# Audio-WestlakeU/SAR-SSL

Hardware: AMD Instinct MI355X
Metric: pretrain_segments_per_sec (higher is better)
Workload: dtype fp16 stem + f32 residual stream (fp16-pair MFMA operands: hi hi + lo hi + hi lo), bf16 backward

## Files before the change

sar-ssl_amd/csrc/conv3x3.hip:

```cpp
#include "common.h"
#include <stdlib.h>

#define TR 8
#define TCOL 64
#define HR (TR + 2)
#define HC (TCOL + 2)
#define NPIX_H (HR * HC)
#define NCHUNK_H (NPIX_H * 8)
#define X_ITERS 11
#define W_ELEMS (9 * 64 * 64)
#define X_ELEMS (NPIX_H * 64)
#define Y_ELEMS (TR * TCOL * 64)

struct ConvArgs {
    const void* in; const void* w; void* out;
    float* acc_ws; int acc_in, acc_out;
    const float* scale; const float* shift; int prologue;
    int nb, F, T;
    int part_in, part_w;
    double* stats;
    const void* bn_y;
    const float* bn_aff;
    int prio;
    const float* c1_w;
// ... 655 lines not shown
    volatile __attribute__((address_space(3))) unsigned* ready3 = (volatile __attribute__((address_space(3))) unsigned*)&sReady[half];
    for (int it = 0; it < nrounds; ++it) {
        const int tile = tile_of(it);
        if (tile >= ntiles) break;
        const TileCoord tc = coord(tile);
        while (*ready3 < (unsigned)(it + 1) * 4u) __builtin_amdgcn_s_sleep(1);
        asm volatile("" ::: "memory");

        f32x16 acc[2][2];
#pragma unroll
        for (int i = 0; i < 2; ++i)
#pragma unroll
            for (int j = 0; j < 2; ++j)
#pragma unroll
                for (int r = 0; r < 16; ++r) acc[i][j][r] = 0.f;
        {
            bf16x8 wf[2][2], xf[2][2];
            auto fetch = [&](int s, int buf) {
                const int tap = s >> 2, kc = s & 3;
                const int kh = tap / 3, kw = tap - kh * 3;
#pragma unroll
                for (int i = 0; i < 2; ++i) wf[buf][i] = *(const bf16x8*)(sW + laneW[kc] + (tap * 64 + i * 32) * 64);
#pragma unroll
                for (int j = 0; j < 2; ++j) xf[buf][j] = *(const bf16x8*)(sX + laneX[kw][kc] + ((kh + j) * PHC) * 64);
            };
            if (a.prio) __builtin_amdgcn_s_setprio(3);
            fetch(0, 0);
#pragma unroll
            for (int s = 0; s < 36; ++s) {
                const int cur = s & 1;
                if (s + 1 < 36) fetch(s + 1, cur ^ 1);
                __builtin_amdgcn_sched_barrier(0);
#pragma unroll
                for (int i = 0; i < 2; ++i)
#pragma unroll
                    for (int j = 0; j < 2; ++j)
                        acc[i][j] = mfma16<bf16>(wf[cur][i], xf[cur][j], acc[i][j]);
            }
            if (a.prio) __builtin_amdgcn_s_setprio(0);
        }
        __builtin_amdgcn_s_waitcnt(0x0F70);
        uint2 av[2];
        bool pv[2];
#pragma unroll
        for (int j = 0; j < 2; ++j) {
            const int f = tc.f0 + 2 * hw + j, t = tc.t0 + (lane & 31);
            pv[j] = f < F && t < Tn;
            av[j] = *(const uint2*)((const uint16_t*)a.c1_a0 + (((long)tc.b * F + min(f, F - 1)) * Tn + min(t, Tn - 1)) * 4);
        }
        half_barrier(cnt, epoch, lane);
        uint16_t* stg = sX + hw * (64 * 64);
        __builtin_amdgcn_s_waitcnt(0x0F70);
        if constexpr (!__is_same(TY, bf16)) {
#pragma unroll
            for (int j = 0; j < 2; ++j) {
                av[j].x = pack2_bf16(H16<TY>::lo(av[j].x), H16<TY>::hi(av[j].x));
                av[j].y = pack2_bf16(H16<TY>::lo(av[j].y), H16<TY>::hi(av[j].y));
            }
        }
        uint16_t* a0t = sX + 4 * (64 * 64) + hw * 256;
        {
            const int j = lane >> 5;
            const uint2 q = j ? av[1] : av[0];
            uint16_t* d = a0t + j * 32 + (lane & 31);
            d[0] = (uint16_t)(q.x & 0xffffu); d[64] = (uint16_t)(q.x >> 16); d[128] = (uint16_t)(q.y & 0xffffu); d[192] = (uint16_t)(q.y >> 16);
        }
#pragma unroll
        for (int i = 0; i < 2; ++i) {
            const bf16x8 wfr = *(const bf16x8*)&sC1[(i * 32 + (lane & 31)) * 16 + (lane >> 5) * 8];
#pragma unroll
            for (int j = 0; j < 2; ++j) {
                union { uint4 u; bf16x8 b; } bx;
                bx.u = make_uint4(av[j].x, av[j].y, 0x00003f80u, 0u);
                f32x16 y;
#pragma unroll
                for (int r = 0; r < 16; ++r) y[r] = 0.f;
                y = __builtin_amdgcn_mfma_f32_32x32x16_bf16(wfr, bx.b, y, 0, 0, 0);
#pragma unroll
                for (int r = 0; r < 16; ++r) acc[i][j][r] = (y[r] > 0.f && pv[j]) ? acc[i][j][r] : 0.f;
            }
        }
#pragma unroll
        for (int i = 0; i < 2; ++i)
#pragma unroll
            for (int g = 0; g < 4; ++g)
#pragma unroll
                for (int j = 0; j < 2; ++j) {
                    uint2 w2;
                    w2.x = pack2_bf16(acc[i][j][g * 4 + 0], acc[i][j][g * 4 + 1]);
                    w2.y = pack2_bf16(acc[i][j][g * 4 + 2], acc[i][j][g * 4 + 3]);
                    *(uint2*)(stg + swz(j * 32 + (lane & 31), i * 4 + g) + 4 * (lane >> 5)) = w2;
                }
        __builtin_amdgcn_s_waitcnt(0xC07F);
        __builtin_amdgcn_wave_barrier();
        f32x16 d2[2];
#pragma unroll
        for (int nb = 0; nb < 2; ++nb)
#pragma unroll
            for (int r = 0; r < 16; ++r) d2[nb][r] = 0.f;
        const int m = lane & 31;
#pragma unroll
        for (int ks = 0; ks < 4; ++ks) {
            union { uint4 u; bf16x8 b; } ax;
            ax.u = *(const uint4*)(a0t + min(m, 3) * 64 + ks * 16 + (lane >> 5) * 8);
            if (m == 4) ax.u = make_uint4(0x3f803f80u, 0x3f803f80u, 0x3f803f80u, 0x3f803f80u);
            else if (m > 4) ax.u = make_uint4(0u, 0u, 0u, 0u);
#pragma unroll
            for (int nb = 0; nb < 2; ++nb)
                d2[nb] = __builtin_amdgcn_mfma_f32_32x32x16_bf16(ax.b, tr_frag(stg, ks * 16, nb * 32, lane), d2[nb], 0, 0, 0);
        }
#pragma unroll
        for (int nb = 0; nb < 2; ++nb)
#pragma unroll
            for (int r = 0; r < 4; ++r) gacc[nb][r] += d2[nb][r];
        __builtin_amdgcn_s_waitcnt(0xC07F);
        if (lane == 0) atomicAdd(&sFree[half], 1u);
    }
    __syncthreads();
    if (a.clk && blockIdx.x == 0 && tid == 0) { a.clk[2] = __builtin_amdgcn_s_memtime(); a.clk[3] = __builtin_amdgcn_s_memrealtime(); }
    float* fold = (float*)sW + 1024;
#pragma unroll
    for (int nb = 0; nb < 2; ++nb) {
        const int co = nb * 32 + (lane & 31);
        if (lane < 32) {
#pragma unroll
            for (int r = 0; r < 4; ++r) fold[wave * 320 + co * 4 + r] = gacc[nb][r];
        } else fold[wave * 320 + 256 + co] = gacc[nb][0];
    }
    __syncthreads();
    for (int q = tid; q < 320; q += 512) {
        float s = 0.f;
#pragma unroll
        for (int w = 0; w < 8; ++w) s += fold[w * 320 + q];
        atomicAdd(&a.c1_red[q < 256 ? q : 512 + (q - 256)], (double)s);
    }
}

struct WgradArgs {
    const void* dy;
    const void* zin;
    const float* scale; const float* shift; int prologue;
    float* partial;
    int nb, F, T;
    int part_dy, part_z;
    const float* c1_w;
    const void* y;
    const float* aff;
    const double* red;
    int use_stats;
    void* dy_out;
    const void* dy4;
    const float* W4;
    float* pg_w4; float* pg_gamma; float* pg_beta;
};
enum { DY_LOAD = 0, DY_APPLY = 1, DY_C4 = 2 };

__device__ __forceinline__ int swzc(int p, int col, int chunk) { return (p * 8 + (chunk ^ (((col >> 1) & 1) << 2))) * 8; }
__device__ __forceinline__ bf16x8 tr_pair(const uint16_t* p0, const uint16_t* p1) {
    typedef __attribute__((ext_vector_type(4))) short s16x4;
    union { s16x4 v[2]; bf16x8 b; } u;
    u.v[0] = __builtin_amdgcn_ds_read_tr16_b64_v4i16((__attribute__((address_space(3))) s16x4*)p0);
    u.v[1] = __builtin_amdgcn_ds_read_tr16_b64_v4i16((__attribute__((address_space(3))) s16x4*)p1);
    return u.b;
}

__global__ __launch_bounds__(512) void conv3x3_wgrad_kernel(WgradArgs a) {
    __shared__ __attribute__((aligned(16))) uint16_t sY[Y_ELEMS];
    __shared__ __attribute__((aligned(16))) uint16_t sX[X_ELEMS];
    const int tid = threadIdx.x, lane = tid & 63, wave = tid >> 6;
    const int wi = wave & 1, wj = (wave >> 1) & 1, wt = wave >> 2;
    const int tap0 = wt ? 5 : 0, ntap = wt ? 4 : 5;
    const int F = a.F, Tn = a.T;
    const int tiles_f = (F + TR - 1) / TR, tiles_t = (Tn + TCOL - 1) / TCOL;
    const int ntiles = a.nb * tiles_f * tiles_t;
    const float* zin = (const float*)a.zin;
    const float* dy = (const float*)a.dy;
    const int cch = tid & 7;

    f32x16 acc[5];
#pragma unroll
    for (int t9 = 0; t9 < 5; ++t9)
#pragma unroll
        for (int r = 0; r < 16; ++r) acc[t9][r] = 0.f;

    int baseA[2], baseB[5][2];
    {
        const int chA = wi * 32 + 16 * ((lane >> 4) & 1) + (lane & 3) * 4, chB = wj * 32 + 16 * ((lane >> 4) & 1) + (lane & 3) * 4;
#pragma unroll
        for (int h = 0; h < 2; ++h) {
            const int loff = (lane >> 5) * 8 + h * 4 + ((lane & 15) >> 2);
            baseA[h] = swzc(loff, loff, chA >> 3) + (chA & 7);
#pragma unroll
            for (int tt = 0; tt < 5; ++tt) {
                const int tap = tap0 + (tt < ntap ? tt : 0);
                const int kh = tap / 3, kw = tap - kh * 3;
                baseB[tt][h] = swzc(kh * HC + kw + loff, kw + loff, chB >> 3) + (chB & 7);
            }
        }
    }

    Chunk<float> rz[X_ITERS], ry[8];
    const int pc = tid >> 3;
    auto issue_loads = [&](int tile) {
        const TileCoord tc = tile_coord(tile, tiles_f, tiles_t);
        const int t = tc.t0 - 1 + pc;
#pragma unroll
        for (int i = 0; i < HR; ++i) rz[i] = load_chunk_clamped<float>(zin, tc.b, tc.f0 - 1 + i, t, F, Tn, cch * 8);
        {
            const int hr = pc >> 1, te = tc.t0 + TCOL - 1 + (pc & 1);
            rz[HR] = load_chunk_clamped<float>(zin, tc.b, tc.f0 - 1 + hr, te, F, Tn, cch * 8);
        }
        const int ty = tc.t0 + pc;
#pragma unroll
        for (int i = 0; i < 8; ++i) ry[i] = load_chunk_clamped<float>(dy, tc.b, tc.f0 + i, ty, F, Tn, cch * 8);
    };
    auto write_tile = [&](int tile) {
        const TileCoord tc = tile_coord(tile, tiles_f, tiles_t);
        float sc[8], sh[8];
#pragma unroll
        for (int e = 0; e < 8; ++e) { sc[e] = a.prologue ? a.scale[cch * 8 + e] : 1.f; sh[e] = a.prologue ? a.shift[cch * 8 + e] : 0.f; }
        const int t = tc.t0 - 1 + pc;
        const bool tv = t >= 0 && t < Tn;
#pragma unroll
        for (int i = 0; i < HR; ++i) {
            const int f = tc.f0 - 1 + i;
            *(uint4*)&sX[swzc(i * HC + pc, pc, cch)] = xform_chunk<float>(rz[i], tv && f >= 0 && f < F, a.prologue, sc, sh, a.part_z);
        }
        if (tid < 160) {
            const int hr = pc >> 1, f = tc.f0 - 1 + hr, te = tc.t0 + TCOL - 1 + (pc & 1);
            *(uint4*)&sX[swzc(hr * HC + TCOL + (pc & 1), TCOL + (pc & 1), cch)] = xform_chunk<float>(rz[HR], f >= 0 && f < F && te < Tn, a.prologue, sc, sh, a.part_z);
        }
        const int ty = tc.t0 + pc;
#pragma unroll
        for (int i = 0; i < 8; ++i)
            *(uint4*)&sY[swzc(i * 64 + pc, pc, cch)] = xform_chunk<float>(ry[i], tc.f0 + i < F && ty < Tn, 0, sc, sh, a.part_dy);
    };

    const int nrounds = (ntiles + gridDim.x - 1) / gridDim.x;
    if (xcd_tile(0, blockIdx.x, gridDim.x) < ntiles) issue_loads(xcd_tile(0, blockIdx.x, gridDim.x));
    for (int it = 0; it < nrounds; ++it) {
        const int tile = xcd_tile(it, blockIdx.x, gridDim.x);
        if (tile >= ntiles) break;
        write_tile(tile);
        __syncthreads();
        const int next = (it + 1 < nrounds) ? xcd_tile(it + 1, blockIdx.x, gridDim.x) : ntiles;
        if (next < ntiles) issue_loads(next);
#pragma unroll 1
        for (int r = 0; r < TR; ++r) {
            const uint16_t* ya[2] = {sY + baseA[0] + r * (64 * 64), sY + baseA[1] + r * (64 * 64)};
            const uint16_t* xb[5][2];
#pragma unroll
            for (int tt = 0; tt < 5; ++tt) { xb[tt][0] = sX + baseB[tt][0] + r * (HC * 64); xb[tt][1] = sX + baseB[tt][1] + r * (HC * 64); }
#pragma unroll
            for (int cb = 0; cb < 4; ++cb) {
                const int co_ = cb * 16 * 64;
                const bf16x8 fa = tr_pair(ya[0] + co_, ya[1] + co_);
                bf16x8 fb[2];
                fb[0] = tr_pair(xb[0][0] + co_, xb[0][1] + co_);
#pragma unroll
                for (int tt = 0; tt < 5; ++tt) {
                    if (tt + 1 < 5 && tt + 1 < ntap) fb[(tt + 1) & 1] = tr_pair(xb[tt + 1][0] + co_, xb[tt + 1][1] + co_);
                    __builtin_amdgcn_sched_barrier(0);
                    if (tt < ntap) acc[tt] = __builtin_amdgcn_mfma_f32_32x32x16_bf16(fa, fb[tt & 1], acc[tt], 0, 0, 0);
                }
            }
        }
        __syncthreads();
    }
    float* P = a.partial + (long)blockIdx.x * W_ELEMS;
#pragma unroll
    for (int tt = 0; tt < 5; ++tt) {
        if (tt < ntap) {
            const int tap = tap0 + tt;
#pragma unroll
            for (int r = 0; r < 16; ++r) {
                const int co = wi * 32 + (r & 3) + 8 * (r >> 2) + 4 * (lane >> 5);
                const int ci = wj * 32 + (lane & 31);
                P[(tap * 64 + co) * 64 + ci] = acc[tt][r];
            }
        }
    }
}

#define WTC 32
#define WHC (WTC + 2)
#define WX_ELEMS (HR * WHC * 64)
#define WY_ELEMS (TR * WTC * 64)
template <bool C1IN = false, typename TA = bf16, int DYSRC = DY_LOAD, typename TY = bf16>
__global__ __launch_bounds__(1024) void conv3x3_wgrad_ws_kernel(WgradArgs a) {
    typedef bf16 T;
    __shared__ __attribute__((aligned(16))) uint16_t sYb[2][WY_ELEMS];
    __shared__ __attribute__((aligned(16))) uint16_t sXb[2][WX_ELEMS];
    constexpr int KROWS = DYSRC == DY_C4 ? 8 : 5, KZ = KROWS * 64;
    static_assert(sizeof(C1Const) == 40 * sizeof(float), "C1Const layout");
    __shared__ __attribute__((aligned(16))) float sK[DYSRC == DY_LOAD ? 4 : KZ + (C1IN ? 8 * 40 : 2 * 64)];
    const int lane = threadIdx.x & 63;
    const int wave_all = __builtin_amdgcn_readfirstlane(threadIdx.x >> 6);
    const bool producer = wave_all >= 8;
    const int tid = threadIdx.x & 511;
    const int wave = wave_all & 7;
    const int wi = wave & 1, wj = (wave >> 1) & 1, wt = wave >> 2;
    const int tap0 = wt ? 5 : 0, ntap = wt ? 4 : 5;
    const int F = a.F, Tn = a.T;
    const int tiles_f = (F + TR - 1) / TR, tiles_t = (Tn + WTC - 1) / WTC;
    const int ntiles = a.nb * tiles_f * tiles_t;
    const TA* zin = (const TA*)a.zin;
    const T* dy = (const T*)a.dy;
    const int cch = tid & 7;

    const int nrounds = (ntiles + gridDim.x - 1) / gridDim.x;
    int tile = xcd_tile(0, blockIdx.x, gridDim.x);
    if (producer) {
        float sc[8], sh[8];
        C1Const kc1;
        if constexpr (DYSRC == DY_LOAD) {
    #pragma unroll
            for (int e = 0; e < 8; ++e) { sc[e] = a.prologue ? a.scale[cch * 8 + e] : 1.f; sh[e] = a.prologue ? a.shift[cch * 8 + e] : 0.f; }
            if (C1IN) c1_setup(kc1, a.c1_w, a.scale, a.shift, cch * 8);
        }
        auto load_z = [&](int b, int f, int t) __attribute__((always_inline)) {
            Chunk<TA> c;
            if (C1IN) {
                f = min(max(f, 0), F - 1); t = min(max(t, 0), Tn - 1);
                const uint2 q = *(const uint2*)(zin + (((long)b * F + f) * Tn + t) * 4);
                c.u = make_uint4(q.x, q.y, 0u, 0u);
            } else c = load_chunk_clamped<TA>(zin, b, f, t, F, Tn, cch * 8);
            return c;
        };
        auto xform_z = [&](const Chunk<TA>& c, bool ok) __attribute__((always_inline)) { return C1IN ? c1_chunk<TA, bf16>(c.u.x, c.u.y, ok, kc1) : xform_chunk<TA, bf16>(c, ok, a.prologue, sc, sh, 0); };

        Chunk<TA> rz[6]; Chunk<T> ry[4];
        Chunk<TY> rv[4]; uint2 rd[4];
        const int pcol = (tid >> 3) & 31;
        const int pr = __builtin_amdgcn_readfirstlane(tid >> 8);
        const int lbX = swzc(pr * WHC + pcol, pcol, cch), lbY = swzc(pr * WTC + pcol, pcol, cch);
        auto coord = [&](int tile) __attribute__((always_inline)) { TileCoord c; c.t0 = (tile % tiles_t) * WTC; tile /= tiles_t; c.f0 = (tile % tiles_f) * TR; c.b = tile / tiles_f; return c; };
        auto issue_loads = [&](const TileCoord tc) __attribute__((always_inline)) {
            constexpr unsigned PXB = C1IN ? 8u : 128u;
            const char* zimg = (const char*)zin + (long)tc.b * F * (long)Tn * PXB;
            const char* yimg = (const char*)dy + (long)tc.b * F * (long)Tn * 128;
            const unsigned zrow = (unsigned)Tn * PXB, yrow = (unsigned)Tn * 128u;
            const int tz = min(max(tc.t0 - 1 + pcol, 0), Tn - 1), ty = min(tc.t0 + pcol, Tn - 1);
            const unsigned vz = C1IN ? (unsigned)tz * 8u : (unsigned)(tz * 64 + cch * 8) * 2u, vy = (unsigned)(ty * 64 + cch * 8) * 2u;
    #pragma unroll
            for (int k = 0; k < 5; ++k) {
                const int f = min(max(tc.f0 - 1 + pr + 2 * k, 0), F - 1);
                const char* prow = zimg + (unsigned)f * zrow;
                if (C1IN) { const uint2 q = *(const uint2*)(prow + vz); rz[k].u = make_uint4(q.x, q.y, 0u, 0u); }
                else rz[k].u = *(const uint4*)(prow + vz);
            }
            {
                const int q = tid >> 3, hr = q >> 1, te = tc.t0 + WTC - 1 + (q & 1);
                rz[5] = load_z(tc.b, tc.f0 - 1 + hr, te);
            }
            const char* vimg = (const char*)a.y + (long)tc.b * F * (long)Tn * 128;
            const char* dcol = (const char*)a.dy4 + ((long)tc.b * Tn + ty) * (long)F * 8;
    #pragma unroll
            for (int k = 0; k < 4; ++k) {
                const int f = min(tc.f0 + pr + 2 * k, F - 1);
                if constexpr (DYSRC != DY_C4) ry[k].u = *(const uint4*)(yimg + (unsigned)f * yrow + vy);
                if constexpr (DYSRC != DY_LOAD) rv[k].u = *(const uint4*)(vimg + (unsigned)f * yrow + vy);
                if constexpr (DYSRC == DY_C4) rd[k] = *(const uint2*)(dcol + (unsigned)f * 8u);
            }
        };
        auto write_piece = [&](const int piece, const TileCoord tc, uint16_t* __restrict__ sX, uint16_t* __restrict__ sY) __attribute__((always_inline)) {
            if (piece < 2) {
                const int t = tc.t0 - 1 + pcol;
                const bool tv = t >= 0 && t < Tn;
    #pragma unroll
                for (int k = 0; k < 5; ++k) {
                    if ((piece == 0) != (k < 3)) continue;
                    const int f = tc.f0 - 1 + pr + 2 * k;
                    *(uint4*)&sX[lbX + k * (2 * WHC * 64)] = xform_z(rz[k], tv && f >= 0 && f < F);
                    }
                if (piece == 1 && tid < 160) {
                    const int q = tid >> 3, hr = q >> 1, f = tc.f0 - 1 + hr, te = tc.t0 + WTC - 1 + (q & 1);
                    *(uint4*)&sX[swzc(hr * WHC + WTC + (q & 1), WTC + (q & 1), cch)] = xform_z(rz[5], f >= 0 && f < F && te < Tn);
                }
            } else {
                const int ty = tc.t0 + pcol;
                if constexpr (DYSRC == DY_LOAD) {
    #pragma unroll
                    for (int k = 0; k < 4; ++k) {
                        *(uint4*)&sY[lbY + k * (2 * WTC * 64)] = xform_chunk<T>(ry[k], tc.f0 + pr + 2 * k < F && ty < Tn, 0, sc, sh, 0);
                    }
                } else {
                    uint32_t o[4][4];
                    constexpr int NE = DYSRC == DY_C4 ? 2 : 4;
                    auto word = [](const uint4& u, int i) __attribute__((always_inline)) { return i == 0 ? u.x : i == 1 ? u.y : i == 2 ? u.z : u.w; };
    #pragma unroll
                    for (int h = 0; h < 8 / NE; ++h) {
                        const int c0 = cch * 8 + h * NE;
                        __builtin_amdgcn_sched_barrier(0);
                        auto row = [&](int r, float* v) __attribute__((always_inline)) {
                            if constexpr (NE == 4) { const float4 q = *(const float4*)&sK[r * 64 + c0]; v[0] = q.x; v[1] = q.y; v[2] = q.z; v[3] = q.w; }
                            else { const float2 q = *(const float2*)&sK[r * 64 + c0]; v[0] = q.x; v[1] = q.y; }
                        };
                        float kA[NE], kB[NE], kC[NE];
                        if constexpr (DYSRC == DY_APPLY) {
                            float thr[NE], sf[NE];
                            row(0, kA); row(1, kB); row(2, kC); row(3, thr); row(4, sf);
                            unsigned sgn = 0u;
    #pragma unroll
                            for (int e = 0; e < NE; ++e) sgn |= __float_as_uint(sf[e]) << e;
    #pragma unroll
                            for (int k = 0; k < 4; ++k) {
                                float d[NE], y[NE], r[NE];
    #pragma unroll
                                for (int j = 0; j < NE / 2; ++j) {
                                    const uint32_t dw = word(ry[k].u, h * (NE / 2) + j), yw = word(rv[k].u, h * (NE / 2) + j);
                                    d[2 * j] = H16<T>::lo(dw); d[2 * j + 1] = H16<T>::hi(dw);
                                    y[2 * j] = H16<TY>::lo(yw); y[2 * j + 1] = H16<TY>::hi(yw);
                                }
                                bn_bwd_apply_relu<NE>(d, y, kA, kB, kC, thr, sgn, r);
    #pragma unroll
                                for (int j = 0; j < NE / 2; ++j) {
                                    o[k][h * (NE / 2) + j] = pack2_bf16(r[2 * j], r[2 * j + 1]);
                                    asm volatile("" : "+v"(o[k][h * (NE / 2) + j]));
                                }
                            }
                        } else {
                            float w0[NE], w1[NE], w2[NE], w3[NE], s3[NE], h3[NE];
                            row(0, w0); row(1, w1); row(2, w2); row(3, w3); row(4, s3); row(5, h3); row(6, kB); row(7, kC);
    #pragma unroll
                            for (int k = 0; k < 4; ++k) {
                                float y[NE], r[NE];
    #pragma unroll
                                for (int j = 0; j < NE / 2; ++j) {
                                    const uint32_t yw = word(rv[k].u, h * (NE / 2) + j);
                                    y[2 * j] = H16<TY>::lo(yw); y[2 * j + 1] = H16<TY>::hi(yw);
                                }
                                const float4 d4 = make_float4(H16<T>::lo(rd[k].x), H16<T>::hi(rd[k].x), H16<T>::lo(rd[k].y), H16<T>::hi(rd[k].y));
                                stem_c4_bwd_apply<NE>(y, d4, w0, w1, w2, w3, s3, h3, s3, kB, kC, r);
    #pragma unroll
                                for (int j = 0; j < NE / 2; ++j) {
                                    o[k][h * (NE / 2) + j] = pack2_bf16(r[2 * j], r[2 * j + 1]);
                                    asm volatile("" : "+v"(o[k][h * (NE / 2) + j]));
                                }
                            }
                        }
                    }
                    char* oimg = (char*)a.dy_out + (long)tc.b * F * (long)Tn * 128;
                    const unsigned yrow = (unsigned)Tn * 128u, vy = (unsigned)(ty * 64 + cch * 8) * 2u;
    #pragma unroll
                    for (int k = 0; k < 4; ++k) {
                        const int f = tc.f0 + pr + 2 * k;
                        const bool ok = f < F && ty < Tn;
                        const uint4 u = ok ? make_uint4(o[k][0], o[k][1], o[k][2], o[k][3]) : make_uint4(0, 0, 0, 0);
                        *(uint4*)&sY[lbY + k * (2 * WTC * 64)] = u;
                        if (ok) *(uint4*)(oimg + (unsigned)f * yrow + vy) = u;
                    }
                }
            }
        };
        auto write_tile = [&](const TileCoord tc, uint16_t* __restrict__ sX, uint16_t* __restrict__ sY) __attribute__((always_inline)) {
            if constexpr (DYSRC != DY_LOAD) {
                if constexpr (C1IN) kc1 = *(const C1Const*)&sK[KZ + cch * 40];
                else {
    #pragma unroll
                    for (int e = 0; e < 8; ++e) { sc[e] = sK[KZ + cch * 8 + e]; sh[e] = sK[KZ + 64 + cch * 8 + e]; }
                }
            }
            write_piece(0, tc, sX, sY); write_piece(1, tc, sX, sY); write_piece(2, tc, sX, sY);
        };

        TileCoord tc = coord(tile < ntiles ? tile : 0);
        if (tile < ntiles) issue_loads(tc);
        if constexpr (DYSRC != DY_LOAD) {
            constexpr int RO = DYSRC == DY_C4 ? 256 : 0;
            if (blockIdx.x == 0 && a.pg_gamma) {
                if (DYSRC == DY_C4 && tid < 256) a.pg_w4[tid] += (float)a.red[tid];
                if (tid < 64) { a.pg_beta[tid] += (float)a.red[RO + tid]; a.pg_gamma[tid] += (float)a.red[RO + 64 + tid]; }
            }
            if (tid < 64) {
                const float invN = 1.0f / (float)((long)a.nb * F * Tn);
                const float s_ = a.aff[tid], h_ = a.aff[64 + tid], mu = a.aff[128 + tid], rs = a.aff[192 + tid];
                const float m1 = a.use_stats ? (float)a.red[RO + tid] * invN : 0.f, m2 = a.use_stats ? (float)a.red[RO + 64 + tid] * invN : 0.f;
                float A, B, C;
                bn_bwd_abc(s_, mu, rs, m1, m2, A, B, C);
                if constexpr (DYSRC == DY_APPLY) {
                    bool neg;
                    const float t = bn_relu_thr(s_, h_, neg);
                    sK[tid] = A; sK[64 + tid] = B; sK[128 + tid] = C; sK[192 + tid] = t; sK[256 + tid] = __uint_as_float(neg ? 1u : 0u);
                } else {
    #pragma unroll
                    for (int c = 0; c < 4; ++c) sK[c * 64 + tid] = a.W4[c * 64 + tid];
                    sK[256 + tid] = s_; sK[320 + tid] = h_; sK[384 + tid] = B; sK[448 + tid] = C;
                }
                if constexpr (C1IN) {
                    if (tid < 8) { C1Const k; c1_setup(k, a.c1_w, a.scale, a.shift, tid * 8); *(C1Const*)&sK[KZ + tid * 40] = k; }
                } else { sK[KZ + tid] = a.prologue ? a.scale[tid] : 1.f; sK[KZ + 64 + tid] = a.prologue ? a.shift[tid] : 0.f; }
            }
            __syncthreads();
        }
        if (tile < ntiles) write_tile(tc, sXb[0], sYb[0]);
        int next = (1 < nrounds) ? xcd_tile(1, blockIdx.x, gridDim.x) : ntiles;
        TileCoord tcn = coord(next < ntiles ? next : 0);
        if (next < ntiles) issue_loads(tcn);
        __syncthreads();
        int cur = 0;
        for (int it = 0; it < nrounds; ++it) {
            if (tile >= ntiles) break;
            if (next < ntiles) write_tile(tcn, sXb[cur ^ 1], sYb[cur ^ 1]);
            const int nn = (it + 2 < nrounds) ? xcd_tile(it + 2, blockIdx.x, gridDim.x) : ntiles;
            const TileCoord tcnn = coord(nn < ntiles ? nn : 0);
            if (nn < ntiles) issue_loads(tcnn);
            __syncthreads();
            cur ^= 1; tile = next; next = nn; tcn = tcnn;
        }
        return;
    }
    f32x16 acc[5];
#pragma unroll
    for (int t9 = 0; t9 < 5; ++t9)
#pragma unroll
        for (int r = 0; r < 16; ++r) acc[t9][r] = 0.f;

    int baseA[2], baseB[5][2];
    {
        const int chA = wi * 32 + 16 * ((lane >> 4) & 1) + (lane & 3) * 4, chB = wj * 32 + 16 * ((lane >> 4) & 1) + (lane & 3) * 4;
#pragma unroll
        for (int h = 0; h < 2; ++h) {
            const int loff = (lane >> 5) * 8 + h * 4 + ((lane & 15) >> 2);
            baseA[h] = swzc(loff, loff, chA >> 3) + (chA & 7);
#pragma unroll
            for (int tt = 0; tt < 5; ++tt) {
                const int tap = tap0 + (tt < ntap ? tt : 0);
                const int kh = tap / 3, kw = tap - kh * 3;
                baseB[tt][h] = swzc(kh * WHC + kw + loff, kw + loff, chB >> 3) + (chB & 7);
            }
        }
    }
    if constexpr (DYSRC != DY_LOAD) __syncthreads();
    __syncthreads();
    int cur = 0;
    for (int it = 0; it < nrounds; ++it) {
        if (tile >= ntiles) break;
        const int next = (it + 1 < nrounds) ? xcd_tile(it + 1, blockIdx.x, gridDim.x) : ntiles;
        const uint16_t* sX = sXb[cur];
        const uint16_t* sY = sYb[cur];
#pragma unroll
        for (int r = 0; r < TR; ++r) {
            const uint16_t* ya[2] = {sY + baseA[0] + r * (WTC * 64), sY + baseA[1] + r * (WTC * 64)};
            const uint16_t* xb[5][2];
#pragma unroll
            for (int tt = 0; tt < 5; ++tt) { xb[tt][0] = sX + baseB[tt][0] + r * (WHC * 64); xb[tt][1] = sX + baseB[tt][1] + r * (WHC * 64); }
#pragma unroll
            for (int cb = 0; cb < WTC / 16; ++cb) {
                const int co_ = cb * 16 * 64;
                const bf16x8 fa = tr_pair(ya[0] + co_, ya[1] + co_);
                bf16x8 fb[2];
                fb[0] = tr_pair(xb[0][0] + co_, xb[0][1] + co_);
#pragma unroll
                for (int tt = 0; tt < 5; ++tt) {
                    if (tt + 1 < 5 && tt + 1 < ntap) fb[(tt + 1) & 1] = tr_pair(xb[tt + 1][0] + co_, xb[tt + 1][1] + co_);
                    __builtin_amdgcn_sched_barrier(0);
                    if (tt < ntap) acc[tt] = __builtin_amdgcn_mfma_f32_32x32x16_bf16(fa, fb[tt & 1], acc[tt], 0, 0, 0);
                }
            }
        }
        __syncthreads();
        cur ^= 1; tile = next;
    }
    float* P = a.partial + (long)blockIdx.x * W_ELEMS;
#pragma unroll
    for (int tt = 0; tt < 5; ++tt) {
        if (tt < ntap) {
            const int tap = tap0 + tt;
#pragma unroll
            for (int r = 0; r < 16; ++r) {
                const int co = wi * 32 + (r & 3) + 8 * (r >> 2) + 4 * (lane >> 5);
                const int ci = wj * 32 + (lane & 31);
                P[(tap * 64 + co) * 64 + ci] = acc[tt][r];
            }
        }
    }
}

__global__ __launch_bounds__(256) void wgrad_reduce_kernel(const float* __restrict__ partial, int nparts, float* __restrict__ dW,
                                                           int accumulate, float* __restrict__ grad_oihw = nullptr) {
    __shared__ float sred[4][64];
    const int col = threadIdx.x & 63, slot = threadIdx.x >> 6;
    const int e = blockIdx.x * 64 + col;
    float s0 = 0.f, s1 = 0.f, s2 = 0.f, s3 = 0.f;
    int p = slot;
    for (; p + 12 < nparts; p += 16) {
        s0 += partial[(long)p * W_ELEMS + e]; s1 += partial[(long)(p + 4) * W_ELEMS + e];
        s2 += partial[(long)(p + 8) * W_ELEMS + e]; s3 += partial[(long)(p + 12) * W_ELEMS + e];
    }
    for (; p < nparts; p += 4) s0 += partial[(long)p * W_ELEMS + e];
    sred[slot][col] = (s0 + s1) + (s2 + s3);
    __syncthreads();
    if (slot == 0) {
        const float t = (sred[0][col] + sred[1][col]) + (sred[2][col] + sred[3][col]);
        if (grad_oihw) { const int tap = e >> 12, coci = e & 4095; grad_oihw[coci * 9 + tap] += t; }
        else dW[e] = accumulate ? dW[e] + t : t;
    }
}

static int conv_cus_override() { const sarssl_ctx* c = sarssl_current(); return c ? c->conv_cus_bwd : 0; }
static int conv_cus(int kind) {
    const int ncu = sarssl_cu_count();
    const int ovr = conv_cus_override();
    if (kind == 1 && ovr > 0) return ovr < ncu ? ovr : ncu;
    return kind == 1 && ncu >= 64 ? (ncu * 7 / 8) & ~7 : ncu;
}
static unsigned long long* conv_clk() { const sarssl_ctx* c = sarssl_current(); return c ? c->conv_clk : nullptr; }
extern "C" long sarssl_wall_clock_khz() {
    int khz = 0;
    if (hipDeviceGetAttribute(&khz, hipDeviceAttributeWallClockRate, 0) != hipSuccess) return 0;
    return (long)khz;
}
static int conv_persistent_grid(int nunits, int kind) {
    const int cus = conv_cus(kind);
    if (nunits <= cus) return nunits;
    const int rounds = (nunits + cus - 1) / cus;
    int g = (nunits + rounds - 1) / rounds;
    g = (g + 7) & ~7;
    return g < cus ? g : cus;
}
static int wgrad_db_grid(int nb, int F, int T) {
    const int ntiles = nb * ((F + TR - 1) / TR) * ((T + WTC - 1) / WTC);
    return conv_persistent_grid(ntiles, 1);
}
static int conv_grid(int nb, int F, int T) {
    int ntiles = nb * ((F + TR - 1) / TR) * ((T + TCOL - 1) / TCOL);
    const int ncu = sarssl_cu_count();
    return ntiles < ncu ? ntiles : ncu;
}
static int conv_npairs(int nb, int F, int T) { return (nb * ((F + TR - 1) / TR) * ((T + PTC - 1) / PTC) + 1) / 2; }
static ConvArgs conv_args(const void* in, const void* w, void* out, int nb, int F, int T, int clk_slot) {
    ConvArgs a = {};
#ifdef CONV_STAMPS
    a.stamps = g_conv_stamps_host;
#endif
    a.prio = (sarssl_mfma_prio() == 1 || sarssl_mfma_prio() == 2);
    a.clk = conv_clk() ? conv_clk() + 4 * clk_slot : nullptr;
    a.in = in; a.w = w; a.out = out;
    a.nb = nb; a.F = F; a.T = T;
    return a;
}

static int conv3x3_launch(const void* in, const void* w, void* out, int dtype, int w_dtype, int nb, int F, int T,
                          const float* scale, const float* shift, int precise, float* ws, double* stats, const void* bn_y,
                          const float* bn_aff, void* stream, int y_dtype = SARSSL_BF16);

extern "C" int sarssl_conv3x3_fwd(const void* in, const void* w, void* out, int dtype, int w_dtype, int nb, int F, int T,
                                  const float* scale, const float* shift, int precise, float* ws, double* stats, void* stream) {
    return conv3x3_launch(in, w, out, dtype, w_dtype, nb, F, T, scale, shift, precise, ws, stats, nullptr, nullptr, stream);
}

extern "C" int sarssl_conv3x3_dgrad_bnred(const void* dy, const void* w, void* dz, int nb, int F, int T, const void* y,
                                          const float* aff, double* red, int y_dtype, void* stream) {
    SARSSL_REQUIRE(y != nullptr && aff != nullptr && red != nullptr && (y_dtype == SARSSL_BF16 || y_dtype == SARSSL_F16), "sarssl_conv3x3_dgrad_bnred");
    return conv3x3_launch(dy, w, dz, SARSSL_BF16, SARSSL_BF16, nb, F, T, nullptr, nullptr, 0, nullptr, red, y, aff, stream, y_dtype);
}

extern "C" int sarssl_conv3x3_fwd_c1(const void* a0, const float* W1, const float* scale, const float* shift, const void* w, void* out,
                                     int nb, int F, int T, double* stats, int dtype, void* stream) {
    SARSSL_REQUIRE(nb > 0 && F > 0 && T > 0 && a0 && W1 && scale && shift && (dtype == SARSSL_BF16 || dtype == SARSSL_F16), "sarssl_conv3x3_fwd_c1");
    if (stats && SARSSL_ZERO(stats, 128 * sizeof(double), (hipStream_t)stream) != hipSuccess) { sarssl_set_error("memset"); return -2; }
    ConvArgs a = conv_args(a0, w, out, nb, F, T, 3);
    a.stats = stats;
    a.scale = scale; a.shift = shift; a.prologue = 1; a.c1_w = W1;
    const int g = conv_persistent_grid(conv_npairs(nb, F, T), 0);
    if (dtype == SARSSL_F16) conv3x3_fwd_pp_kernel<false, true, f16><<<g, 512, 0, (hipStream_t)stream>>>(a);
    else conv3x3_fwd_pp_kernel<false, true><<<g, 512, 0, (hipStream_t)stream>>>(a);
    SARSSL_CHECK_LAUNCH("conv3x3_fwd_pp_kernel<c1in>");
    return 0;
}

extern "C" int sarssl_conv3x3_dgrad_c1red(const void* dy, const void* w, const void* a0, const float* W1, const float* scale,
                                          const float* shift, int nb, int F, int T, double* red, int a0_dtype, void* stream) {
    SARSSL_REQUIRE(nb > 0 && F > 0 && T > 0 && dy && w && a0 && W1 && scale && shift && red && (a0_dtype == SARSSL_BF16 || a0_dtype == SARSSL_F16),
                   "sarssl_conv3x3_dgrad_c1red");
    if (SARSSL_ZERO(red, 644 * sizeof(double), (hipStream_t)stream) != hipSuccess) { sarssl_set_error("memset"); return -2; }
    ConvArgs a = conv_args(dy, w, nullptr, nb, F, T, 4);
    a.scale = scale; a.shift = shift; a.c1_w = W1; a.c1_a0 = a0; a.c1_red = red;
    const int g = conv_persistent_grid(conv_npairs(nb, F, T), 1);
    if (a0_dtype == SARSSL_F16) conv3x3_dgrad_c1red_ws_kernel<f16><<<g, 768, 0, (hipStream_t)stream>>>(a);
    else conv3x3_dgrad_c1red_ws_kernel<bf16><<<g, 768, 0, (hipStream_t)stream>>>(a);
    SARSSL_CHECK_LAUNCH("conv3x3_dgrad_c1red_ws_kernel");
    return 0;
}

static int conv3x3_launch(const void* in, const void* w, void* out, int dtype, int w_dtype, int nb, int F, int T,
                          const float* scale, const float* shift, int precise, float* ws, double* stats, const void* bn_y,
                          const float* bn_aff, void* stream, int y_dtype) {
    SARSSL_REQUIRE(nb > 0 && F > 0 && T > 0, "sarssl_conv3x3_fwd");
    SARSSL_REQUIRE(stats == nullptr || dtype == SARSSL_BF16 || dtype == SARSSL_F16, "sarssl_conv3x3_fwd(fused statistics: 16-bit storage only)");
    if (stats && SARSSL_ZERO(stats, 128 * sizeof(double), (hipStream_t)stream) != hipSuccess) { sarssl_set_error("memset"); return -2; }
    ConvArgs a = conv_args(in, w, out, nb, F, T, bn_y ? 2 : (scale != nullptr ? 0 : 1));
    a.bn_y = bn_y; a.bn_aff = bn_aff;
    a.stats = stats;
    a.scale = scale; a.shift = shift; a.prologue = (scale != nullptr);
    hipStream_t st = (hipStream_t)stream;
    if (dtype == w_dtype && (dtype == SARSSL_BF16 || dtype == SARSSL_F16)) {
        const int g = conv_persistent_grid(conv_npairs(nb, F, T), scale != nullptr ? 0 : 1);
        if (dtype == SARSSL_F16) {
            SARSSL_REQUIRE(bn_y == nullptr, "sarssl_conv3x3_fwd(fp16: forward launches only)");
            conv3x3_fwd_pp_kernel<false, false, f16><<<g, 512, 0, st>>>(a);
        } else if (bn_y && y_dtype == SARSSL_F16) conv3x3_fwd_pp_kernel<true, false, bf16, f16><<<g, 512, 0, st>>>(a);
        else if (bn_y) conv3x3_fwd_pp_kernel<true><<<g, 512, 0, st>>>(a);
        else conv3x3_fwd_pp_kernel<false><<<g, 512, 0, st>>>(a);
    } else if (dtype == SARSSL_F32 && w_dtype == SARSSL_F32) {
        const int grid = conv_grid(nb, F, T);
        if (!precise) conv3x3_fwd_kernel<<<grid, 512, 0, st>>>(a);
        else {
            SARSSL_REQUIRE(ws != nullptr, "sarssl_conv3x3_fwd(precise needs workspace)");
            a.acc_ws = ws;
            ConvArgs p = a;
            p.part_in = 0; p.part_w = 1; p.acc_in = 0; p.acc_out = 1; conv3x3_fwd_kernel<<<grid, 512, 0, st>>>(p);
            p.part_in = 1; p.part_w = 0; p.acc_in = 1; p.acc_out = 1; conv3x3_fwd_kernel<<<grid, 512, 0, st>>>(p);
            p.part_in = 0; p.part_w = 0; p.acc_in = 1; p.acc_out = 0; conv3x3_fwd_kernel<<<grid, 512, 0, st>>>(p);
        }
    } else { sarssl_set_error("sarssl_conv3x3_fwd: unsupported dtypes (%d,%d)", dtype, w_dtype); return -1; }
    SARSSL_CHECK_LAUNCH("conv3x3_fwd_kernel");
    return 0;
}

extern "C" long sarssl_conv3x3_wgrad_workspace_bytes(int nb, int F, int T) {
    const int g1 = conv_grid(nb, F, T), g2 = wgrad_db_grid(nb, F, T);
    return (long)(g1 > g2 ? g1 : g2) * W_ELEMS * sizeof(float);
}

template <typename T, typename TD>
__global__ void conv_taps_kernel(const float* __restrict__ W, T* __restrict__ fwd, TD* __restrict__ dgr) {
    const int e = blockIdx.x * blockDim.x + threadIdx.x;
    if (e >= 9 * 4096) return;
    const int tap = e >> 12, a = (e >> 6) & 63, b = e & 63;
    st_f(fwd + e, W[(a * 64 + b) * 9 + tap]);
    st_f(dgr + e, W[(b * 64 + a) * 9 + (8 - tap)]);
}
extern "C" int sarssl_conv_taps(const float* W, void* fwd, void* dgr, int dtype, void* stream) {
    if (dtype == SARSSL_BF16) conv_taps_kernel<bf16, bf16><<<144, 256, 0, (hipStream_t)stream>>>(W, (bf16*)fwd, (bf16*)dgr);
    else if (dtype == SARSSL_MIX16) conv_taps_kernel<f16, bf16><<<144, 256, 0, (hipStream_t)stream>>>(W, (f16*)fwd, (bf16*)dgr);
    else if (dtype == SARSSL_F32) conv_taps_kernel<float, float><<<144, 256, 0, (hipStream_t)stream>>>(W, (float*)fwd, (float*)dgr);
    else { sarssl_set_error("sarssl_conv_taps: unsupported dtype %d", dtype); return -1; }
    SARSSL_CHECK_LAUNCH("conv_taps_kernel");
    return 0;
}
template <typename T>
__global__ void patch_w_kernel(const float* __restrict__ W, T* __restrict__ out, int d, int F) {
    const long e = (long)blockIdx.x * blockDim.x + threadIdx.x;
    if (e >= (long)d * F * 4) return;
    const int c = e & 3; const long of = e >> 2; const int f = of % F; const long o = of / F;
    st_f(out + e, W[(o * 4 + c) * F + f]);
}
extern "C" int sarssl_patch_w(const float* W, void* out, int d, int F, int dtype, void* stream) {
    const long n = (long)d * F * 4;
    if (dtype == SARSSL_BF16) patch_w_kernel<bf16><<<(int)((n + 255) / 256), 256, 0, (hipStream_t)stream>>>(W, (bf16*)out, d, F);
    else if (dtype == SARSSL_F32) patch_w_kernel<float><<<(int)((n + 255) / 256), 256, 0, (hipStream_t)stream>>>(W, (float*)out, d, F);
    else if (dtype == SARSSL_F16) patch_w_kernel<f16><<<(int)((n + 255) / 256), 256, 0, (hipStream_t)stream>>>(W, (f16*)out, d, F);
    else { sarssl_set_error("sarssl_patch_w: unsupported dtype %d", dtype); return -1; }
    SARSSL_CHECK_LAUNCH("patch_w_kernel");
    return 0;
}
__global__ void patch_wgrad_accum_kernel(const float* __restrict__ g, int nslice, float* __restrict__ grad, int d, int F) {
    const long e = (long)blockIdx.x * blockDim.x + threadIdx.x;
    const long n = (long)d * F * 4;
    if (e >= n) return;
    float s = 0.f;
    for (int k = 0; k < nslice; ++k) s += g[k * n + e];
    const int c = e & 3; const long of = e >> 2; const int f = of % F; const long o = of / F;
    grad[(o * 4 + c) * F + f] += s;
}
extern "C" int sarssl_patch_wgrad_accum(const float* g, int nslice, float* grad, int d, int F, void* stream) {
    SARSSL_REQUIRE(nslice > 0, "sarssl_patch_wgrad_accum");
    const long n = (long)d * F * 4;
    patch_wgrad_accum_kernel<<<(int)((n + 255) / 256), 256, 0, (hipStream_t)stream>>>(g, nslice, grad, d, F);
    SARSSL_CHECK_LAUNCH("patch_wgrad_accum_kernel");
    return 0;
}

template <bool C1IN>
static void wgrad_bf16_launch(const WgradArgs& a, int g2, hipStream_t st, bool z_f16) {
    if (z_f16) conv3x3_wgrad_ws_kernel<C1IN, f16><<<g2, 1024, 0, st>>>(a);
    else conv3x3_wgrad_ws_kernel<C1IN><<<g2, 1024, 0, st>>>(a);
}

extern "C" int sarssl_conv3x3_wgrad(const void* dy, const void* zin, int dtype, int nb, int F, int T,
                                    const float* scale, const float* shift, float* dW, float* partial, int precise,
                                    void* stream) {
    SARSSL_REQUIRE(nb > 0 && F > 0 && T > 0, "sarssl_conv3x3_wgrad");
    WgradArgs a = {};
    a.dy = dy; a.zin = zin; a.scale = scale; a.shift = shift; a.prologue = (scale != nullptr);
    a.partial = partial; a.nb = nb; a.F = F; a.T = T; a.part_dy = 0; a.part_z = 0;
    hipStream_t st = (hipStream_t)stream;
    const int grid = conv_grid(nb, F, T);
    const int rblocks = W_ELEMS / 64;
    if (dtype == SARSSL_BF16 || dtype == SARSSL_MIX16) {
        const int g2 = wgrad_db_grid(nb, F, T);
        wgrad_bf16_launch<false>(a, g2, st, dtype == SARSSL_MIX16);
        wgrad_reduce_kernel<<<rblocks, 256, 0, st>>>(partial, g2, dW, 0);
    } else if (dtype == SARSSL_F32) {
        const int npass = precise ? 3 : 1;
        for (int pass = 0; pass < npass; ++pass) {
            WgradArgs p = a;
            if (precise) { p.part_dy = (pass == 1); p.part_z = (pass == 0); }
            conv3x3_wgrad_kernel<<<grid, 512, 0, st>>>(p);
            wgrad_reduce_kernel<<<rblocks, 256, 0, st>>>(partial, grid, dW, pass > 0);
        }
    } else { sarssl_set_error("sarssl_conv3x3_wgrad: unsupported dtype %d", dtype); return -1; }
    SARSSL_CHECK_LAUNCH("conv3x3_wgrad_kernel");
    return 0;
}

extern "C" int sarssl_conv3x3_wgrad_acc(const void* dy, const void* zin, int nb, int F, int T, const float* scale, const float* shift,
                                        float* grad_oihw, float* partial, int z_dtype, void* stream) {
    SARSSL_REQUIRE(nb > 0 && F > 0 && T > 0 && grad_oihw && partial && (z_dtype == SARSSL_BF16 || z_dtype == SARSSL_F16), "sarssl_conv3x3_wgrad_acc");
    WgradArgs a = {};
    a.dy = dy; a.zin = zin; a.scale = scale; a.shift = shift; a.prologue = (scale != nullptr);
    a.partial = partial; a.nb = nb; a.F = F; a.T = T; a.part_dy = 0; a.part_z = 0;
    hipStream_t st = (hipStream_t)stream;
    const int g2 = wgrad_db_grid(nb, F, T);
    wgrad_bf16_launch<false>(a, g2, st, z_dtype == SARSSL_F16);
    wgrad_reduce_kernel<<<W_ELEMS / 64, 256, 0, st>>>(partial, g2, nullptr, 0, grad_oihw);
    SARSSL_CHECK_LAUNCH("conv3x3_wgrad_kernel(acc)");
    return 0;
}
extern "C" int sarssl_conv3x3_wgrad_c1_acc(const void* dy, const void* a0, const float* W1, int nb, int F, int T, const float* scale,
                                           const float* shift, float* grad_oihw, float* partial, int a0_dtype, void* stream) {
    SARSSL_REQUIRE(nb > 0 && F > 0 && T > 0 && grad_oihw && partial && W1 && scale && shift && (a0_dtype == SARSSL_BF16 || a0_dtype == SARSSL_F16),
                   "sarssl_conv3x3_wgrad_c1_acc");
    WgradArgs a = {};
    a.dy = dy; a.zin = a0; a.scale = scale; a.shift = shift; a.prologue = 1; a.c1_w = W1;
    a.partial = partial; a.nb = nb; a.F = F; a.T = T;
    hipStream_t st = (hipStream_t)stream;
    const int g2 = wgrad_db_grid(nb, F, T);
    wgrad_bf16_launch<true>(a, g2, st, a0_dtype == SARSSL_F16);
    wgrad_reduce_kernel<<<W_ELEMS / 64, 256, 0, st>>>(partial, g2, nullptr, 0, grad_oihw);
    SARSSL_CHECK_LAUNCH("conv3x3_wgrad_ws_kernel<c1in>");
    return 0;
}

extern "C" int sarssl_conv3x3_wgrad_c4_acc(const void* y3, const void* dy4, const float* W4, const float* aff3, const double* red, int use_stats,
                                           const void* y2, const float* scale, const float* shift, int nb, int F, int T, void* dy3_out,
                                           float* grad_oihw, float* partial, float* gW4, float* dgamma, float* dbeta, int y_dtype, void* stream) {
    SARSSL_REQUIRE(nb > 0 && F > 0 && T > 0 && y3 && dy4 && W4 && aff3 && red && y2 && dy3_out && grad_oihw && partial &&
                   (y_dtype == SARSSL_BF16 || y_dtype == SARSSL_F16), "sarssl_conv3x3_wgrad_c4_acc");
    SARSSL_REQUIRE((scale == nullptr) == (shift == nullptr), "sarssl_conv3x3_wgrad_c4_acc");
    SARSSL_REQUIRE((gW4 == nullptr) == (dgamma == nullptr) && (gW4 == nullptr) == (dbeta == nullptr), "sarssl_conv3x3_wgrad_c4_acc");
    SARSSL_REQUIRE(dy3_out != y3 && dy3_out != y2, "sarssl_conv3x3_wgrad_c4_acc");
    WgradArgs a = {};
    a.zin = y2; a.scale = scale; a.shift = shift; a.prologue = (scale != nullptr);
    a.partial = partial; a.nb = nb; a.F = F; a.T = T;
    a.y = y3; a.dy4 = dy4; a.W4 = W4; a.aff = aff3; a.red = red; a.use_stats = use_stats; a.dy_out = dy3_out;
    a.pg_w4 = gW4; a.pg_gamma = dgamma; a.pg_beta = dbeta;
    hipStream_t st = (hipStream_t)stream;
    const int g2 = wgrad_db_grid(nb, F, T);
    if (y_dtype == SARSSL_F16) conv3x3_wgrad_ws_kernel<false, f16, DY_C4, f16><<<g2, 1024, 0, st>>>(a);
    else conv3x3_wgrad_ws_kernel<false, bf16, DY_C4, bf16><<<g2, 1024, 0, st>>>(a);
    wgrad_reduce_kernel<<<W_ELEMS / 64, 256, 0, st>>>(partial, g2, nullptr, 0, grad_oihw);
    SARSSL_CHECK_LAUNCH("conv3x3_wgrad_ws_kernel<c4>");
    return 0;
}
extern "C" int sarssl_conv3x3_wgrad_c1_apply_acc(const void* dz, const void* y, const float* aff, const double* red, int use_stats, void* dy_out,
                                                 const void* a0, const float* W1, const float* scale, const float* shift, int nb, int F, int T,
                                                 float* grad_oihw, float* partial, float* dgamma, float* dbeta, int y_dtype, void* stream) {
    SARSSL_REQUIRE(nb > 0 && F > 0 && T > 0 && dz && y && aff && red && dy_out && a0 && W1 && scale && shift && grad_oihw && partial &&
                   (y_dtype == SARSSL_BF16 || y_dtype == SARSSL_F16), "sarssl_conv3x3_wgrad_c1_apply_acc");
    SARSSL_REQUIRE((dgamma == nullptr) == (dbeta == nullptr), "sarssl_conv3x3_wgrad_c1_apply_acc");
    SARSSL_REQUIRE(dy_out != y && dy_out != a0, "sarssl_conv3x3_wgrad_c1_apply_acc");
    WgradArgs a = {};
    a.dy = dz; a.zin = a0; a.scale = scale; a.shift = shift; a.prologue = 1; a.c1_w = W1;
    a.partial = partial; a.nb = nb; a.F = F; a.T = T;
    a.y = y; a.aff = aff; a.red = red; a.use_stats = use_stats; a.dy_out = dy_out;
    a.pg_gamma = dgamma; a.pg_beta = dbeta;
    hipStream_t st = (hipStream_t)stream;
    const int g2 = wgrad_db_grid(nb, F, T);
    if (y_dtype == SARSSL_F16) conv3x3_wgrad_ws_kernel<true, f16, DY_APPLY, f16><<<g2, 1024, 0, st>>>(a);
    else conv3x3_wgrad_ws_kernel<true, bf16, DY_APPLY, bf16><<<g2, 1024, 0, st>>>(a);
    wgrad_reduce_kernel<<<W_ELEMS / 64, 256, 0, st>>>(partial, g2, nullptr, 0, grad_oihw);
    SARSSL_CHECK_LAUNCH("conv3x3_wgrad_ws_kernel<c1in, apply>");
    return 0;
}
```

Baseline: 6050.

## Interleave next-tile global loads with LDS writes in wgrad producer waves

The producer waves of the warp-specialized wgrad kernel used to issue all of the next tile's global loads in one block after writing the current tile to LDS. The loads are now split into z and dy groups, and each group is issued right after the matching LDS write piece retires its registers. This spreads memory traffic across the producer's work and reduces register pressure from holding two tiles' loads at once. The change also adds optional s_memtime timestamp instrumentation, compiled only under CONV_STAMPS, and restructures the loop and early-exit sync handling.

```diff
diff --git a/sar-ssl_amd/csrc/conv3x3.hip b/sar-ssl_amd/csrc/conv3x3.hip
--- a/sar-ssl_amd/csrc/conv3x3.hip
+++ b/sar-ssl_amd/csrc/conv3x3.hip
@@ -831,7 +831,15 @@
     const void* dy4;
     const float* W4;
     float* pg_w4; float* pg_gamma; float* pg_beta;
+#ifdef CONV_STAMPS
+    unsigned long long* stamps;
+#endif
 };
+#ifdef CONV_STAMPS
+#define WSTAMP(k) do { if (blockIdx.x == 0 && it < 8 && lane == 0 && a.stamps) a.stamps[(wave_all * 8 + it) * 12 + (k)] = __builtin_amdgcn_s_memtime(); } while (0)
+#else
+#define WSTAMP(k) do {} while (0)
+#endif
 enum { DY_LOAD = 0, DY_APPLY = 1, DY_C4 = 2 };
 
 __device__ __forceinline__ int swzc(int p, int col, int chunk) { return (p * 8 + (chunk ^ (((col >> 1) & 1) << 2))) * 8; }
@@ -992,6 +1000,7 @@
     if (producer) {
         float sc[8], sh[8];
         C1Const kc1;
+        int it = 8;
         if constexpr (DYSRC == DY_LOAD) {
     #pragma unroll
             for (int e = 0; e < 8; ++e) { sc[e] = a.prologue ? a.scale[cch * 8 + e] : 1.f; sh[e] = a.prologue ? a.shift[cch * 8 + e] : 0.f; }
@@ -1014,24 +1023,30 @@
         const int pr = __builtin_amdgcn_readfirstlane(tid >> 8);
         const int lbX = swzc(pr * WHC + pcol, pcol, cch), lbY = swzc(pr * WTC + pcol, pcol, cch);
         auto coord = [&](int tile) __attribute__((always_inline)) { TileCoord c; c.t0 = (tile % tiles_t) * WTC; tile /= tiles_t; c.f0 = (tile % tiles_f) * TR; c.b = tile / tiles_f; return c; };
-        auto issue_loads = [&](const TileCoord tc) __attribute__((always_inline)) {
+        auto issue_z = [&](const TileCoord tc, const int grp) __attribute__((always_inline)) {
             constexpr unsigned PXB = C1IN ? 8u : 128u;
             const char* zimg = (const char*)zin + (long)tc.b * F * (long)Tn * PXB;
-            const char* yimg = (const char*)dy + (long)tc.b * F * (long)Tn * 128;
-            const unsigned zrow = (unsigned)Tn * PXB, yrow = (unsigned)Tn * 128u;
-            const int tz = min(max(tc.t0 - 1 + pcol, 0), Tn - 1), ty = min(tc.t0 + pcol, Tn - 1);
-            const unsigned vz = C1IN ? (unsigned)tz * 8u : (unsigned)(tz * 64 + cch * 8) * 2u, vy = (unsigned)(ty * 64 + cch * 8) * 2u;
+            const unsigned zrow = (unsigned)Tn * PXB;
+            const int tz = min(max(tc.t0 - 1 + pcol, 0), Tn - 1);
+            const unsigned vz = C1IN ? (unsigned)tz * 8u : (unsigned)(tz * 64 + cch * 8) * 2u;
     #pragma unroll
             for (int k = 0; k < 5; ++k) {
+                if ((grp == 0) != (k < 3)) continue;
                 const int f = min(max(tc.f0 - 1 + pr + 2 * k, 0), F - 1);
                 const char* prow = zimg + (unsigned)f * zrow;
                 if (C1IN) { const uint2 q = *(const uint2*)(prow + vz); rz[k].u = make_uint4(q.x, q.y, 0u, 0u); }
                 else rz[k].u = *(const uint4*)(prow + vz);
             }
-            {
+            if (grp == 1) {
                 const int q = tid >> 3, hr = q >> 1, te = tc.t0 + WTC - 1 + (q & 1);
                 rz[5] = load_z(tc.b, tc.f0 - 1 + hr, te);
             }
+        };
+        auto issue_dy = [&](const TileCoord tc) __attribute__((always_inline)) {
+            const char* yimg = (const char*)dy + (long)tc.b * F * (long)Tn * 128;
+            const unsigned yrow = (unsigned)Tn * 128u;
+            const int ty = min(tc.t0 + pcol, Tn - 1);
+            const unsigned vy = (unsigned)(ty * 64 + cch * 8) * 2u;
             const char* vimg = (const char*)a.y + (long)tc.b * F * (long)Tn * 128;
             const char* dcol = (const char*)a.dy4 + ((long)tc.b * Tn + ty) * (long)F * 8;
     #pragma unroll
@@ -1042,7 +1057,7 @@
                 if constexpr (DYSRC == DY_C4) rd[k] = *(const uint2*)(dcol + (unsigned)f * 8u);
             }
         };
-        auto write_piece = [&](const int piece, const TileCoord tc, uint16_t* __restrict__ sX, uint16_t* __restrict__ sY) __attribute__((always_inline)) {
+        auto write_piece = [&](const int piece, const TileCoord tc, uint16_t* __restrict__ sX, uint16_t* __restrict__ sY, const TileCoord tcl) __attribute__((always_inline)) {
             if (piece < 2) {
                 const int t = tc.t0 - 1 + pcol;
                 const bool tv = t >= 0 && t < Tn;
@@ -1056,6 +1071,7 @@
                     const int q = tid >> 3, hr = q >> 1, f = tc.f0 - 1 + hr, te = tc.t0 + WTC - 1 + (q & 1);
                     *(uint4*)&sX[swzc(hr * WHC + WTC + (q & 1), WTC + (q & 1), cch)] = xform_z(rz[5], f >= 0 && f < F && te < Tn);
                 }
+                issue_z(tcl, piece);
             } else {
                 const int ty = tc.t0 + pcol;
                 if constexpr (DYSRC == DY_LOAD) {
@@ -1063,6 +1079,7 @@
                     for (int k = 0; k < 4; ++k) {
                         *(uint4*)&sY[lbY + k * (2 * WTC * 64)] = xform_chunk<T>(ry[k], tc.f0 + pr + 2 * k < F && ty < Tn, 0, sc, sh, 0);
                     }
+                    issue_dy(tcl);
                 } else {
                     uint32_t o[4][4];
                     constexpr int NE = DYSRC == DY_C4 ? 2 : 4;
@@ -1119,6 +1136,9 @@
                             }
                         }
                     }
+                    WSTAMP(3);
+                    issue_dy(tcl);
+                    WSTAMP(5);
                     char* oimg = (char*)a.dy_out + (long)tc.b * F * (long)Tn * 128;
                     const unsigned yrow = (unsigned)Tn * 128u, vy = (unsigned)(ty * 64 + cch * 8) * 2u;
     #pragma unroll
@@ -1129,10 +1149,11 @@
                         *(uint4*)&sY[lbY + k * (2 * WTC * 64)] = u;
                         if (ok) *(uint4*)(oimg + (unsigned)f * yrow + vy) = u;
                     }
+                    WSTAMP(4);
                 }
             }
         };
-        auto write_tile = [&](const TileCoord tc, uint16_t* __restrict__ sX, uint16_t* __restrict__ sY) __attribute__((always_inline)) {
+        auto write_tile = [&](const TileCoord tc, uint16_t* __restrict__ sX, uint16_t* __restrict__ sY, const TileCoord tcl) __attribute__((always_inline)) {
             if constexpr (DYSRC != DY_LOAD) {
                 if constexpr (C1IN) kc1 = *(const C1Const*)&sK[KZ + cch * 40];
                 else {
@@ -1140,11 +1161,22 @@
                     for (int e = 0; e < 8; ++e) { sc[e] = sK[KZ + cch * 8 + e]; sh[e] = sK[KZ + 64 + cch * 8 + e]; }
                 }
             }
-            write_piece(0, tc, sX, sY); write_piece(1, tc, sX, sY); write_piece(2, tc, sX, sY);
+#ifdef CONV_STAMPS
+            asm volatile("" : "+v"(rz[0].u.x));
+#endif
+            WSTAMP(1);
+            write_piece(0, tc, sX, sY, tcl); write_piece(1, tc, sX, sY, tcl);
+            WSTAMP(2);
+            write_piece(2, tc, sX, sY, tcl);
         };
 
-        TileCoord tc = coord(tile < ntiles ? tile : 0);
-        if (tile < ntiles) issue_loads(tc);
+        if (tile >= ntiles) {
+            if constexpr (DYSRC != DY_LOAD) __syncthreads();
+            __syncthreads();
+            return;
+        }
+        const TileCoord tc = coord(tile);
+        issue_z(tc, 0); issue_z(tc, 1); issue_dy(tc);
         if constexpr (DYSRC != DY_LOAD) {
             constexpr int RO = DYSRC == DY_C4 ? 256 : 0;
             if (blockIdx.x == 0 && a.pg_gamma) {
@@ -1172,21 +1204,21 @@
             }
             __syncthreads();
         }
-        if (tile < ntiles) write_tile(tc, sXb[0], sYb[0]);
         int next = (1 < nrounds) ? xcd_tile(1, blockIdx.x, gridDim.x) : ntiles;
         TileCoord tcn = coord(next < ntiles ? next : 0);
-        if (next < ntiles) issue_loads(tcn);
+        write_tile(tc, sXb[0], sYb[0], tcn);
         __syncthreads();
         int cur = 0;
-        for (int it = 0; it < nrounds; ++it) {
-            if (tile >= ntiles) break;
-            if (next < ntiles) write_tile(tcn, sXb[cur ^ 1], sYb[cur ^ 1]);
+        for (it = 0; next < ntiles; ++it) {
+            WSTAMP(0);
             const int nn = (it + 2 < nrounds) ? xcd_tile(it + 2, blockIdx.x, gridDim.x) : ntiles;
             const TileCoord tcnn = coord(nn < ntiles ? nn : 0);
-            if (nn < ntiles) issue_loads(tcnn);
+            write_tile(tcn, sXb[cur ^ 1], sYb[cur ^ 1], tcnn);
             __syncthreads();
-            cur ^= 1; tile = next; next = nn; tcn = tcnn;
-        }
+            WSTAMP(6);
+            cur ^= 1; next = nn; tcn = tcnn;
+        }
+        __syncthreads();
         return;
     }
     f32x16 acc[5];
@@ -1218,6 +1250,7 @@
         const int next = (it + 1 < nrounds) ? xcd_tile(it + 1, blockIdx.x, gridDim.x) : ntiles;
         const uint16_t* sX = sXb[cur];
         const uint16_t* sY = sYb[cur];
+        WSTAMP(0);
 #pragma unroll
         for (int r = 0; r < TR; ++r) {
             const uint16_t* ya[2] = {sY + baseA[0] + r * (WTC * 64), sY + baseA[1] + r * (WTC * 64)};
@@ -1238,7 +1271,9 @@
                 }
             }
         }
+        WSTAMP(1);
         __syncthreads();
+        WSTAMP(2);
         cur ^= 1; tile = next;
     }
     float* P = a.partial + (long)blockIdx.x * W_ELEMS;
@@ -1452,6 +1487,13 @@
     return 0;
 }
 
+static WgradArgs wgrad_args() {
+    WgradArgs a = {};
+#ifdef CONV_STAMPS
+    a.stamps = g_conv_stamps_host;
+#endif
+    return a;
+}
 template <bool C1IN>
 static void wgrad_bf16_launch(const WgradArgs& a, int g2, hipStream_t st, bool z_f16) {
     if (z_f16) conv3x3_wgrad_ws_kernel<C1IN, f16><<<g2, 1024, 0, st>>>(a);
@@ -1462,7 +1504,7 @@
                                     const float* scale, const float* shift, float* dW, float* partial, int precise,
                                     void* stream) {
     SARSSL_REQUIRE(nb > 0 && F > 0 && T > 0, "sarssl_conv3x3_wgrad");
-    WgradArgs a = {};
+    WgradArgs a = wgrad_args();
     a.dy = dy; a.zin = zin; a.scale = scale; a.shift = shift; a.prologue = (scale != nullptr);
     a.partial = partial; a.nb = nb; a.F = F; a.T = T; a.part_dy = 0; a.part_z = 0;
     hipStream_t st = (hipStream_t)stream;
@@ -1488,7 +1530,7 @@
 extern "C" int sarssl_conv3x3_wgrad_acc(const void* dy, const void* zin, int nb, int F, int T, const float* scale, const float* shift,
                                         float* grad_oihw, float* partial, int z_dtype, void* stream) {
     SARSSL_REQUIRE(nb > 0 && F > 0 && T > 0 && grad_oihw && partial && (z_dtype == SARSSL_BF16 || z_dtype == SARSSL_F16), "sarssl_conv3x3_wgrad_acc");
-    WgradArgs a = {};
+    WgradArgs a = wgrad_args();
     a.dy = dy; a.zin = zin; a.scale = scale; a.shift = shift; a.prologue = (scale != nullptr);
     a.partial = partial; a.nb = nb; a.F = F; a.T = T; a.part_dy = 0; a.part_z = 0;
     hipStream_t st = (hipStream_t)stream;
@@ -1502,7 +1544,7 @@
                                            const float* shift, float* grad_oihw, float* partial, int a0_dtype, void* stream) {
     SARSSL_REQUIRE(nb > 0 && F > 0 && T > 0 && grad_oihw && partial && W1 && scale && shift && (a0_dtype == SARSSL_BF16 || a0_dtype == SARSSL_F16),
                    "sarssl_conv3x3_wgrad_c1_acc");
-    WgradArgs a = {};
+    WgradArgs a = wgrad_args();
     a.dy = dy; a.zin = a0; a.scale = scale; a.shift = shift; a.prologue = 1; a.c1_w = W1;
     a.partial = partial; a.nb = nb; a.F = F; a.T = T;
     hipStream_t st = (hipStream_t)stream;
@@ -1521,7 +1563,7 @@
     SARSSL_REQUIRE((scale == nullptr) == (shift == nullptr), "sarssl_conv3x3_wgrad_c4_acc");
     SARSSL_REQUIRE((gW4 == nullptr) == (dgamma == nullptr) && (gW4 == nullptr) == (dbeta == nullptr), "sarssl_conv3x3_wgrad_c4_acc");
     SARSSL_REQUIRE(dy3_out != y3 && dy3_out != y2, "sarssl_conv3x3_wgrad_c4_acc");
-    WgradArgs a = {};
+    WgradArgs a = wgrad_args();
     a.zin = y2; a.scale = scale; a.shift = shift; a.prologue = (scale != nullptr);
     a.partial = partial; a.nb = nb; a.F = F; a.T = T;
     a.y = y3; a.dy4 = dy4; a.W4 = W4; a.aff = aff3; a.red = red; a.use_stats = use_stats; a.dy_out = dy3_out;
@@ -1541,7 +1583,7 @@
                    (y_dtype == SARSSL_BF16 || y_dtype == SARSSL_F16), "sarssl_conv3x3_wgrad_c1_apply_acc");
     SARSSL_REQUIRE((dgamma == nullptr) == (dbeta == nullptr), "sarssl_conv3x3_wgrad_c1_apply_acc");
     SARSSL_REQUIRE(dy_out != y && dy_out != a0, "sarssl_conv3x3_wgrad_c1_apply_acc");
-    WgradArgs a = {};
+    WgradArgs a = wgrad_args();
     a.dy = dz; a.zin = a0; a.scale = scale; a.shift = shift; a.prologue = 1; a.c1_w = W1;
     a.partial = partial; a.nb = nb; a.F = F; a.T = T;
     a.y = y; a.aff = aff; a.red = red; a.use_stats = use_stats; a.dy_out = dy_out;
```

Result: no change. 6098, median of 6 (+0.8%).
